# svohr/mixemt

Measured on AMD Instinct MI355X. Metric: read x hap cells/sec through the EM iteration (EM iters/sec reported beside it as em_iters_per_s), 1000000 reads x 5408 haps in total, whole job, higher is better.
Workload: dtype f64

## Files before the change

mixemt_amd/_lib.py:

```python

import ctypes
import os

_PKG = os.path.dirname(os.path.abspath(__file__))
LIB_PATH = os.environ.get("MXM_LIB") or os.path.join(_PKG, "lib", "libmixemt_hip.so")

c_i32, c_i64, c_f64 = ctypes.c_int32, ctypes.c_int64, ctypes.c_double
c_ptr, c_size = ctypes.c_void_p, ctypes.c_size_t


class EmState(ctypes.Structure):
    _fields_ = [("done", c_i32), ("iters", c_i32), ("l1", c_f64), ("ticket", ctypes.c_uint32), ("error", ctypes.c_uint32)]


class Coded(ctypes.Structure):
    _fields_ = [("rec", c_ptr), ("rec_off", c_ptr), ("ndist", c_ptr), ("R", c_i64),
                ("P_rest", c_ptr), ("ldp_rest", c_i64), ("w_rest", c_ptr), ("R_rest", c_i64),
                ("wide_rows", c_ptr), ("n_wide", c_i64),
                ("qrec", c_ptr), ("qoff", c_ptr), ("nquad", c_ptr), ("quad_rows", c_ptr), ("n_quad_rows", c_i64),
                ("byte_rows", c_ptr), ("n_byte_rows", c_i64)]


class SampleTile(ctypes.Structure):
    _fields_ = [("sample", c_i32), ("count", c_i32), ("first", c_i64)]
# ... 140 lines not shown
    "mxm_gather_columns": (ctypes.c_int, [c_ptr, c_i64, c_i64, c_i32, c_ptr, c_i32, c_ptr, c_i64, c_ptr]),
    "mxm_fold_logaddexp": (ctypes.c_int, [c_ptr, c_i64, ctypes.POINTER(c_ptr), ctypes.POINTER(c_i64), c_i32,
                                          c_i64, c_i32, c_f64, c_ptr]),
}

FINISH_SIGNATURES = {
    "mxm_samples_finish_workspace_bytes": (c_size, [c_i64, c_i32, c_i32]),
    "mxm_votes_samples": (ctypes.c_int, [ctypes.POINTER(Coded), c_ptr, c_i32, c_i32, c_ptr, c_ptr, c_ptr, c_ptr, c_ptr, c_ptr,
                                         c_ptr, c_ptr, c_ptr, c_ptr, c_ptr, c_size, c_ptr]),
    "mxm_gather_columns_samples": (ctypes.c_int, [ctypes.POINTER(Coded), c_ptr, c_i32, c_i32, c_ptr, c_ptr, c_i32, c_ptr,
                                                  c_ptr, c_size, c_ptr]),
    "mxm_em_loop_samples_narrow": (ctypes.c_int, [ctypes.POINTER(Coded), c_ptr, c_i32, c_i32, c_ptr, c_i32, c_ptr, c_ptr,
                                                  c_ptr, c_ptr, c_ptr, c_ptr, c_f64, c_i32, c_i32, c_ptr, c_ptr, c_size,
                                                  c_ptr, ctypes.POINTER(EmState)]),
    "mxm_assign_reads_samples": (ctypes.c_int, [ctypes.POINTER(Coded), c_ptr, c_i32, c_i32, c_ptr, c_i32, c_ptr, c_ptr,
                                                c_ptr, c_ptr, c_ptr, c_ptr, c_f64, c_ptr, c_ptr, c_ptr, c_size, c_ptr]),
}

VARCHECK_SIGNATURES = {
    "mxm_check_variants_samples": (ctypes.c_int, [c_ptr, c_i32, c_i64, c_ptr, c_ptr, c_i32, c_ptr, c_ptr, c_i32, c_i64, c_ptr,
                                                  c_ptr, c_i32, c_f64, c_f64, c_f64, c_i32, c_i32, c_ptr, c_ptr, c_ptr, c_ptr]),
}

ABI_VERSION = 603

PROGRESS_FN = ctypes.CFUNCTYPE(None, ctypes.POINTER(EmState), c_i32, c_ptr)

_lib = None


class MixemtHipError(RuntimeError):
    pass


def load():
    global _lib
    if _lib is not None:
        return _lib
    if not os.path.exists(LIB_PATH):
        raise MixemtHipError(
            "libmixemt_hip.so is not built (%s); run `python -m mixemt_amd.build` -- "
            "there is no CPU fallback for the EM hot path" % LIB_PATH)
    from . import _dev
    lib = ctypes.CDLL(LIB_PATH)
    try:
        lib.mxm_version.restype = ctypes.c_int
        lib.mxm_version.argtypes = []
        have = lib.mxm_version()
    except AttributeError:
        have = None
    if have != ABI_VERSION:
        raise MixemtHipError("%s reports ABI version %s, this binding was written for %d: rebuild with "
                             "`python -m mixemt_amd.build --force`" % (LIB_PATH, have, ABI_VERSION))
    for name, (restype, argtypes) in (list(SIGNATURES.items()) + list(FINISH_SIGNATURES.items())
                                      + list(VARCHECK_SIGNATURES.items())):
        try:
            fn = getattr(lib, name)
        except AttributeError:
            raise MixemtHipError("%s has ABI version %d but lacks %s: rebuild with "
                                 "`python -m mixemt_amd.build --force`" % (LIB_PATH, have, name))
        fn.restype = restype
        fn.argtypes = argtypes
    _lib = lib
    try:
        if _dev.torch is not None and _dev.torch.cuda.is_available():
            lib.mxm_preload()
    except Exception:
        pass
    return lib


def check(rc, what):
    if rc != 0:
        msg = load().mxm_last_error().decode("utf-8", "replace")
        raise ValueError("%s failed (%d): %s" % (what, rc, msg))
```

mixemt_amd/build.py:

```python

import hashlib
import os
import shutil
import subprocess
import sys

_PKG = os.path.dirname(os.path.abspath(__file__))
_ROOT = os.path.dirname(_PKG)
SRC = os.path.join(_PKG, "csrc", "mixemt_hip.hip")
HDRS = [os.path.join(_ROOT, "include", name) for name in ("mixemt_hip.h", "mixemt_hip_tuning.h", "mixemt_hip_samples_finish.h",
                                                           "mixemt_hip_var_check.h")]
LIB_DIR = os.path.join(_PKG, "lib")
LIB = os.path.join(LIB_DIR, "libmixemt_hip.so")
ARCH = "gfx950"


def _hipcc():
    for cand in (os.environ.get("HIPCC"), shutil.which("hipcc"), "/opt/rocm/bin/hipcc"):
        if cand and os.path.exists(cand):
            return cand
    raise RuntimeError("hipcc not found (set HIPCC or add /opt/rocm/bin to PATH)")


def _sources():
    csrc = os.path.dirname(SRC)
    return sorted(os.path.join(csrc, f) for f in os.listdir(csrc) if f.endswith((".hip", ".hpp"))) + HDRS


def _digest(flags):
    h = hashlib.sha256()
    for path in _sources():
        with open(path, "rb") as fin:
            h.update(fin.read())
    h.update(" ".join(flags).encode())
# ... 44 lines not shown
```

mixemt_amd/csrc/build_lut_kernels.hpp:

```cpp
#ifndef MIXEMT_BUILD_LUT_KERNELS_HPP
#define MIXEMT_BUILD_LUT_KERNELS_HPP

#define LUT_THREADS 256
#define LUT_CAP 128
#define LUT_NOMATCH (15u << 3)
#ifndef LUT_CPL
#define LUT_CPL 4
#endif
#ifndef LUT_UNROLL
#define LUT_UNROLL 8
#endif
#ifndef LUT_PIPE
#define LUT_PIPE 0
#endif

template <int NT, int CPL>
__global__ __launch_bounds__(LUT_THREADS) void build_lut_kernel(
    const uint8_t *__restrict__ E, int64_t lde, int64_t e_bytes, const double *__restrict__ lhit,
    const double *__restrict__ lmiss, const uint8_t *__restrict__ obsmap, const int64_t *__restrict__ row_ptr,
    const uint16_t *__restrict__ site, const uint8_t *__restrict__ obs, const int64_t *__restrict__ order,
    int64_t R, int H, double *__restrict__ M, int64_t ldm, int vec_ok, int compact) {
    static_assert(CPL == 4 || CPL == 8, "one 4- or 8-byte table load per lane, site and tile");
    constexpr int EW = CPL / 4;
    __shared__ double s_lut[2][LUT_CAP][16];
    __shared__ uint2 s_rec[2][LUT_CAP];
    const int t = threadIdx.x;
    const auto e_rsrc = __builtin_amdgcn_make_buffer_rsrc(const_cast<uint8_t *>(E), 0, (int)e_bytes, 0x00020000);

    auto stage = [&](int buf, int slot, int64_t at) {
        const uint32_t s0 = site[at];
        const uint32_t oc = obsmap[obs[at]];
        const double hv = lhit[s0], mv = lmiss[s0];
        s_rec[buf][slot] = make_uint2((uint32_t)(s0 * (uint32_t)lde), oc * 0x01010101u);
        d2 *dst = reinterpret_cast<d2 *>(&s_lut[buf][slot][0]);
        dst[0] = d2{hv, mv};
#pragma unroll
        for (int q = 1; q < 8; ++q) dst[q] = d2{mv, mv};
    };

    int cur = 0;
    bool have = false;
    for (int64_t i = blockIdx.x; i < R; i += gridDim.x, cur ^= 1) {
        const int64_t r = order != nullptr ? order[i] : i;
        const int64_t beg = row_ptr[r], end = row_ptr[r + 1];
// ... 117 lines not shown
```

mixemt_amd/csrc/coded_kernels.hpp:

```cpp
#ifndef MIXEMT_CODED_KERNELS_HPP
#define MIXEMT_CODED_KERNELS_HPP

#define ENC_THREADS 256
#define ENC_SLOTS 1024
#define ENC_MAX_CODES 256
#define ENC_MAX_WIDE 1024
#define ENC_WIDE_SLOTS 4096
#define ENC_EMPTY 0xFFFFFFFFFFFFFFFFull

__host__ __device__ __forceinline__ int rec_code_bytes(int nd, int ldc) { return nd > ENC_MAX_CODES ? 2 * ldc : ldc; }
__device__ __forceinline__ int rec_code_at(const uint8_t *codes, int h, bool wide) {
    return wide ? (int)reinterpret_cast<const uint16_t *>(codes)[h] : (int)codes[h];
}

template <int NCH, bool WIDE>
__device__ __forceinline__ void encode_one_row(int64_t r, const double *__restrict__ M, int64_t ldm, int H, int ldc,
                                               uint8_t *__restrict__ rec, int64_t rec_cap, int64_t *__restrict__ rec_off,
                                               int32_t *__restrict__ ndist, double *__restrict__ rowmax,
                                               unsigned long long *__restrict__ stats) {
    constexpr int NW = ENC_THREADS / 64;
    constexpr int SLOTS = WIDE ? ENC_WIDE_SLOTS : ENC_SLOTS;
    constexpr int MAXC = WIDE ? ENC_MAX_WIDE : ENC_MAX_CODES;
    constexpr int SPT = SLOTS / ENC_THREADS;
    __shared__ unsigned long long s_key[SLOTS];
    __shared__ unsigned short s_code[SLOTS];
    __shared__ double s_red[NW];
    __shared__ int s_wcnt[NW];
    __shared__ int s_flag, s_n;
    __shared__ long long s_off;
    const int t = threadIdx.x, lane = t & 63, wv = t >> 6;
    typedef unsigned int u4 __attribute__((ext_vector_type(4)));
    typedef unsigned int u2 __attribute__((ext_vector_type(2)));

    const auto rsrc = __builtin_amdgcn_make_buffer_rsrc(const_cast<double *>(M + r * ldm), 0, H * 8, 0x00020000);
    double x[NCH][4];
#pragma unroll
    for (int k = 0; k < NCH; ++k) {
        const int off = (t + k * ENC_THREADS) * 32;
        const d2 a = __builtin_bit_cast(d2, (u4)__builtin_amdgcn_raw_buffer_load_b128(rsrc, off, 0, 2));
// ... 122 lines not shown
        }
#pragma unroll
        for (int k = 0; k < NCH; ++k) {
            const int c0 = 4 * (t + k * ENC_THREADS);
            if (c0 < ldc) {
                unsigned int cd[4];
#pragma unroll
                for (int e = 0; e < 4; ++e) cd[e] = (c0 + e < H) ? (unsigned int)s_code[slot[k][e]] : 0u;
                if constexpr (WIDE) {
                    u2 word;
                    word.x = cd[0] | (cd[1] << 16);
                    word.y = cd[2] | (cd[3] << 16);
                    reinterpret_cast<u2 *>(rec + off)[t + k * ENC_THREADS] = word;
                } else {
                    reinterpret_cast<unsigned int *>(rec + off)[t + k * ENC_THREADS] =
                        cd[0] | (cd[1] << 8) | (cd[2] << 16) | (cd[3] << 24);
                }
            }
        }
    }
    if (t == 0) {
        if constexpr (WIDE) {
            if (off >= 0) {
                ndist[r] = D;
                rec_off[r] = off;
                atomicAdd(&stats[1], ~0ull);
            }
        } else {
            rowmax[r] = shift;
            ndist[r] = (off >= 0) ? D : 0;
            rec_off[r] = (off >= 0) ? off : 0;
            if (off < 0) atomicAdd(&stats[1], 1ull);
        }
    }
    __syncthreads();
}

template <int NCH>
__global__ __launch_bounds__(ENC_THREADS) void encode_rows_kernel(
    const double *__restrict__ M, int64_t ldm, int64_t R, int H, int ldc, uint8_t *__restrict__ rec, int64_t rec_cap,
    int64_t *__restrict__ rec_off, int32_t *__restrict__ ndist, double *__restrict__ rowmax,
    unsigned long long *__restrict__ stats) {
    for (int64_t r = blockIdx.x; r < R; r += gridDim.x)
        encode_one_row<NCH, false>(r, M, ldm, H, ldc, rec, rec_cap, rec_off, ndist, rowmax, stats);
}

template <int NCH>
__global__ __launch_bounds__(ENC_THREADS) void encode_wide_rows_kernel(
    const double *__restrict__ M, int64_t ldm, int64_t R, int H, int ldc, uint8_t *__restrict__ rec, int64_t rec_cap,
    int64_t *__restrict__ rec_off, int32_t *__restrict__ ndist, double *__restrict__ rowmax,
    unsigned long long *__restrict__ stats) {
    constexpr int CH = 32;
    __shared__ int s_list[CH];
    __shared__ int s_nlist;
    const int t = threadIdx.x;
    const int64_t nchunk = (R + CH - 1) / CH;
    for (int64_t c = blockIdx.x; c < nchunk; c += gridDim.x) {
        if (t == 0) s_nlist = 0;
        __syncthreads();
        const int64_t r = c * CH + t;
        if (t < CH && r < R && ndist[r] == 0) s_list[atomicAdd(&s_nlist, 1)] = t;
        __syncthreads();
        const int n = s_nlist;
        for (int i = 0; i < n; ++i)
            encode_one_row<NCH, true>(c * CH + s_list[i], M, ldm, H, ldc, rec, rec_cap, rec_off, ndist, rowmax, stats);
        __syncthreads();
    }
}

template <int THREADS, int NCH, int NBUF, bool NT, bool RESIDENT, bool WIDE_PREFETCH, bool CHECK = false>
__device__ __forceinline__ void coded_row_pass(const uint8_t *__restrict__ rec, const int64_t *__restrict__ rec_off,
                                               const int32_t *__restrict__ ndist, int ldc, const double *__restrict__ w,
                                               const int64_t *__restrict__ wide_rows, int64_t n_wide, int64_t R,
                                               const double (&p)[NCH][4], double (&acc)[NCH][4], bool &meta_ready,
                                               int *chk_result = nullptr, const int64_t *__restrict__ row_list = nullptr,
                                               int64_t n_list = 0, const int32_t *__restrict__ nquad = nullptr, int vbid = -1,
                                               int vgrid = 0) {
    static_assert(NBUF >= 3, "codes NBUF - 1 rows ahead, tables NBUF - 2");
    constexpr int NW = THREADS / 64;
    constexpr int AUX = NT ? 2 : 0;
    __shared__ double s_tbl[NBUF][ENC_MAX_CODES];
    __shared__ __attribute__((aligned(16))) double red[NBUF][NW];
    const int t = threadIdx.x, lane = t & 63, wv = t >> 6;
    const int nword = ldc >> 2;
    const int64_t bid = vbid >= 0 ? (int64_t)vbid : (int64_t)blockIdx.x, grid = vbid >= 0 ? (int64_t)vgrid : (int64_t)gridDim.x;
    const row_deal deal(row_list != nullptr ? n_list : R, bid, grid);
    const int voff = t * 4;
    int last_w = t + (NCH - 1) * THREADS;
// ... 474 lines not shown
```

mixemt_amd/csrc/mixemt_hip.hip:

```cpp
#include <hip/hip_runtime.h>
#include <stdint.h>
#include <stdio.h>
#include <stdlib.h>
#include <string.h>
#include <math.h>
#include <algorithm>
#include <atomic>
#include <mutex>
#include <type_traits>
#include <utility>
#include <vector>

#include "mixemt_hip.h"
#include "mixemt_hip_tuning.h"

#include "common.hpp"
#include "aln_encode.hpp"
#include "bam_reader.hpp"
#include "coded_kernels.hpp"
#include "quad_kernels.hpp"
#include "quad_batched_kernels.hpp"
#include "build_kernels.hpp"
#include "build_lut_kernels.hpp"
#include "build_sparse_kernels.hpp"
#include "em_kernels.hpp"
#include "estep_kernels.hpp"
#include "aux_kernels.hpp"
#include "records_kernels.hpp"
#include "fused_kernels.hpp"
#include "fused_cols_kernels.hpp"
#include "fused_coded_kernels.hpp"
#include "fused_narrow_kernels.hpp"
#include "samples_kernels.hpp"
#include "samples_finish_kernels.hpp"
#include "exchange.hpp"
#include "aln_walk.hpp"
#include "observe_kernels.hpp"
// ... 141 lines not shown
}

extern "C" int mxm_build_em_matrix(const uint8_t *E, int64_t lde, const double *lhit,
                                   const double *lmiss, const int64_t *row_ptr, const uint16_t *site,
                                   const uint8_t *obs, int64_t R, int32_t H, int32_t S, double *M,
                                   int64_t ldm, void *stream) {
    if (R < 0 || H <= 0 || S <= 0) return fail(-1, "mxm_build_em_matrix: bad shape R=%lld H=%d", (long long)R, H);
    if (lde < (((int64_t)H + 7) & ~(int64_t)7) || (lde & 7) != 0 || (reinterpret_cast<uintptr_t>(E) & 7) != 0)
        return fail(-1, "mxm_build_em_matrix: E must be 8-byte aligned with lde a multiple of 8 and >= H rounded up to 8 (lde=%lld)", (long long)lde);
    if (ldm < H) return fail(-1, "mxm_build_em_matrix: ldm < H");
    if (S > 65536) return fail(-1, "mxm_build_em_matrix: more than 65536 variant sites");
    if (R == 0) return 0;
    const int grid = clamp_grid(R, num_cu() * 8);
    const int vec_ok = ((ldm & 1) == 0) && ((reinterpret_cast<uintptr_t>(M) & 15) == 0);
    hipLaunchKernelGGL(build_em_matrix_kernel, dim3(grid), dim3(BUILD_THREADS), 0, (hipStream_t)stream, E,
                       lde, lhit, lmiss, row_ptr, site, obs, R, (int)H, M, ldm, vec_ok);
    HIP_TRY(hipGetLastError());
    return 0;
}

static int build_lut_impl(const char *who, const uint8_t *Ecode, int64_t lde, const double *lhit,
                          const double *lmiss, const uint8_t *obsmap, const int64_t *row_ptr, const uint16_t *site,
                          const uint8_t *obs, const int64_t *order, int64_t R, int32_t H, int32_t S, double *M, int64_t ldm,
                          int compact, hipStream_t s) {
    if (H > 8192) return fail(-1, "%s: more than 8192 haplogroups (H=%d)%s", who, H, compact ? "" : ": use mxm_build_em_matrix");
    if (lde < (((int64_t)H + 7) & ~(int64_t)7) || (lde & 7) != 0 || (reinterpret_cast<uintptr_t>(Ecode) & 7) != 0)
        return fail(-1, "%s: Ecode must be 8-byte aligned with lde a multiple of 8 and >= H rounded up to 8 (lde=%lld)", who, (long long)lde);
    if (ldm < H) return fail(-1, "%s: ldm < H", who);
    if (S > 65536 || (int64_t)S * lde >= ((int64_t)1 << 31))
        return fail(-1, "%s: table of %d x %lld bytes exceeds one buffer descriptor", who, S, (long long)lde);
    if (R == 0) return 0;
    const int grid = clamp_grid(R, num_cu() * 8);
    const int nt = (H + LUT_THREADS * LUT_CPL - 1) / (LUT_THREADS * LUT_CPL);
    const int vec_ok = ((ldm & 1) == 0) && ((reinterpret_cast<uintptr_t>(M) & 15) == 0);
    const bool ok = dispatch_width<8>(nt, [&](auto n) {
        constexpr int NT = decltype(n)::value;
        hipLaunchKernelGGL((build_lut_kernel<NT, LUT_CPL>), dim3(grid), dim3(LUT_THREADS), 0, s, Ecode, lde, (int64_t)S * lde, lhit,
                           lmiss, obsmap, row_ptr, site, obs, order, R, (int)H, M, ldm, vec_ok, compact);
    });
    if (!ok) return fail(-1, "%s: H=%d outside the kernel's range", who, H);
    HIP_TRY(hipGetLastError());
    return 0;
}

extern "C" int mxm_build_em_matrix_lut(const uint8_t *Ecode, int64_t lde, const double *lhit, const double *lmiss,
                                       const uint8_t *obsmap, const int64_t *row_ptr, const uint16_t *site,
                                       const uint8_t *obs, const int64_t *order, int64_t R, int32_t H, int32_t S,
                                       double *M, int64_t ldm, void *stream) {
    if (R < 0 || H <= 0 || S <= 0) return fail(-1, "mxm_build_em_matrix_lut: bad shape R=%lld H=%d", (long long)R, H);
    return build_lut_impl("mxm_build_em_matrix_lut", Ecode, lde, lhit, lmiss, obsmap, row_ptr, site, obs,
                          order, R, H, S, M, ldm, 0, (hipStream_t)stream);
}

extern "C" int mxm_build_em_matrix_lut_rows(const uint8_t *Ecode, int64_t lde, const double *lhit, const double *lmiss,
                                            const uint8_t *obsmap, const int64_t *row_ptr, const uint16_t *site,
                                            const uint8_t *obs, const int64_t *rows, int64_t n_rows, int32_t H, int32_t S,
                                            double *M_out, int64_t ldm, void *stream) {
    if (n_rows < 0 || H <= 0 || S <= 0 || rows == nullptr) return fail(-1, "mxm_build_em_matrix_lut_rows: bad arguments");
    return build_lut_impl("mxm_build_em_matrix_lut_rows", Ecode, lde, lhit, lmiss, obsmap, row_ptr, site, obs, rows, n_rows, H, S,
                          M_out, ldm, 1, (hipStream_t)stream);
}
// ... 115 lines not shown

extern "C" int mxm_build_em_records(const uint8_t *maj, const double *lhit, const double *lmiss,
                                    const int32_t *mk_ptr, const uint16_t *mk_hap, const uint8_t *mk_base,
                                    const int64_t *row_ptr, const uint16_t *site, const uint8_t *obs,
                                    const int64_t *order, int64_t R, int32_t H, int32_t S, double *M, int64_t ldm,
                                    uint8_t *rec, size_t rec_bytes, int64_t *rec_off, int32_t *ndist, double *rowmax,
                                    int64_t *stats, int64_t *fallback, int64_t *n_fallback, void *stream) {
    MXM_ENTER();
    if (!mxm_linear_supported(H))
        return fail(-1, "mxm_build_em_records: records need H in [65, 8192] (H=%d)", H);
    if (rec == nullptr || (reinterpret_cast<uintptr_t>(rec) & 15) || rec_bytes < (size_t)coded_ld(H) + 16 * ENC_MAX_CODES ||
        rec_off == nullptr || ndist == nullptr || rowmax == nullptr || stats == nullptr)
        return fail(-1, "mxm_build_em_records: record buffer (16-byte aligned, >= one record) and output arrays required");
    spb_records out;
    out.rec = rec;
    out.rec_cap = (long long)rec_bytes;
    out.rec_off = rec_off;
    out.ndist = ndist;
    out.rowmax = rowmax;
    out.stats = reinterpret_cast<unsigned long long *>(stats);
    out.ldc = coded_ld(H);
    return build_sparse_impl("mxm_build_em_records", maj, lhit, lmiss, mk_ptr, mk_hap, mk_base, row_ptr, site, obs, order,
                             R, H, S, M, ldm, &out, fallback, n_fallback, (hipStream_t)stream);
}

template <typename ST>
static int linearize_wide(const double *M, int64_t ldm, int64_t R, int H, ST *P, int64_t ldp, double *rowmax,
                          hipStream_t s) {
    const int nch = (H / 2 + 255) / 256;
    int cap = num_cu() * 2 < MXM_MAX_WG ? num_cu() * 2 : MXM_MAX_WG;
    const int nwg = clamp_grid((R + 1) / 2, cap);
    const bool ok = dispatch_width<16>(nch, [&](auto n) {
        hipLaunchKernelGGL((linearize_wide_kernel<decltype(n)::value, ST>), dim3(nwg), dim3(256), 0, s, M, ldm, R, H, P, ldp, rowmax);
    });
    return ok ? 0 : 1;
}

static inline bool wide_rows_ok(const void *M, int64_t ldm, int H) {
    return ((H & 1) == 0) && ((ldm & 1) == 0) && ((reinterpret_cast<uintptr_t>(M) & 15) == 0) && H >= 64 && H <= 8192;
}

extern "C" int mxm_linearize(const double *M, int64_t ldm, int64_t R, int32_t H, double *P, int64_t ldp,
                             double *rowmax, void *stream) {
    if (R < 0 || H <= 0) return fail(-1, "mxm_linearize: bad shape");
    if (ldm < H || ldp < H || (ldp & 1)) return fail(-1, "mxm_linearize: ldp must be even and >= H (ldp=%lld)", (long long)ldp);
    if (R == 0) return 0;
// ... 2168 lines not shown
```

mixemt_amd/preprocess.py:

```python

import collections
import math
import os
import sys
import time

import numpy

from . import _lib
from . import phylotree
from ._dev import as_device, current_stream, device_empty, require_gpu, to_host, torch

MUT_WT = 0.01
MUT_MAX = 0.5


class _LazyLut(object):

    def __init__(self, expected, n_haps, code_of, obsmap):
        self._expected, self._n_haps, self.code_of = expected, n_haps, code_of
        self._items = {"obsmap": obsmap}

    def __getitem__(self, key):
        if key == "ecode" and "ecode" not in self._items:
# ... 252 lines not shown
    return torch.argsort(keys, stable=True)


def build_em_matrix_device(tables, row_ptr, site, obs, out=None, kernel="auto", sort_rows="auto"):
    lib = _lib.load()
    dev = require_gpu()
    if kernel == "auto":
        kernel = "bytes" if tables.lut() is None else "sparse"
    if kernel not in ("sparse", "lut", "bytes"):
        raise ValueError("kernel must be 'auto', 'sparse', 'lut' or 'bytes'")
    if kernel == "sparse":
        if tables.lut() is None or tables.n_haps > 8192:
            raise ValueError("tables do not qualify for the marker kernel (its leftover rows need the lookup-table kernel)")
        enc = tables.sparse_device()
        row_ptr_d = as_device(row_ptr, torch.int64, dev)
        site_d = as_device(site, torch.uint16, dev)
        obs_d = as_device(obs, torch.uint8, dev)
        n_rows = row_ptr_d.numel() - 1
        n_haps = tables.n_haps
        if out is None:
            out = device_empty((n_rows, n_haps), torch.float64, dev, "the EM input matrix")
        if n_rows == 0:
            return out
        fallback = torch.empty(n_rows, dtype=torch.int64, device=dev)
        n_fallback = torch.zeros(1, dtype=torch.int64, device=dev)
        _lib.check(lib.mxm_build_em_matrix_sparse(
            enc["maj"].data_ptr(), enc["lhit"].data_ptr(), enc["lmiss"].data_ptr(), enc["mk_ptr"].data_ptr(),
            enc["mk_hap"].data_ptr(), enc["mk_base"].data_ptr(), row_ptr_d.data_ptr(), site_d.data_ptr(),
            obs_d.data_ptr(), 0, n_rows, n_haps, len(tables.sites), out.data_ptr(), out.stride(0),
            fallback.data_ptr(), n_fallback.data_ptr(), current_stream()), "mxm_build_em_matrix_sparse")
        left = int(n_fallback.item())
        build_em_matrix_device.last_fallback = left
        if left:
            lut = tables.lut_device()
            rows = fallback[:left].sort().values
            _lib.check(lib.mxm_build_em_matrix_lut(
                lut["ecode"].data_ptr(), lut["ecode"].stride(0), lut["lhit"].data_ptr(), lut["lmiss"].data_ptr(),
                lut["obsmap"].data_ptr(), row_ptr_d.data_ptr(), site_d.data_ptr(), obs_d.data_ptr(),
                rows.data_ptr(), left, n_haps, len(tables.sites), out.data_ptr(), out.stride(0),
                current_stream()), "mxm_build_em_matrix_lut")
        return out
    if kernel == "lut":
        enc = tables.lut_device()
        if enc is None:
            raise ValueError("tables do not qualify for the lookup-table kernel")
        row_ptr_d = as_device(row_ptr, torch.int64, dev)
        site_d = as_device(site, torch.uint16, dev)
        obs_d = as_device(obs, torch.uint8, dev)
        n_rows = row_ptr_d.numel() - 1
        n_haps = tables.n_haps
        if out is None:
            out = device_empty((n_rows, n_haps), torch.float64, dev, "the EM input matrix")
        if n_rows == 0:
            return out
        order = None
        if sort_rows is True or (sort_rows == "auto" and n_rows >= SORT_ROWS_FROM):
            order = row_order_by_position(row_ptr_d, site_d)
        _lib.check(lib.mxm_build_em_matrix_lut(
            enc["ecode"].data_ptr(), enc["ecode"].stride(0), enc["lhit"].data_ptr(), enc["lmiss"].data_ptr(),
            enc["obsmap"].data_ptr(), row_ptr_d.data_ptr(), site_d.data_ptr(), obs_d.data_ptr(),
            0 if order is None else order.data_ptr(), n_rows, n_haps, len(tables.sites),
            out.data_ptr(), out.stride(0), current_stream()), "mxm_build_em_matrix_lut")
        return out
# ... 157 lines not shown
        raise ValueError("records need tables that qualify for the lookup-table kernel and H in [65, 8192]")
    enc = tables.sparse_device()
    lut = tables.lut_device()
    row_ptr_d = as_device(row_ptr, torch.int64, dev)
    site_d = as_device(site, torch.uint16, dev)
    obs_d = as_device(obs, torch.uint8, dev)
    n_rows, n_haps, n_sites = row_ptr_d.numel() - 1, tables.n_haps, len(tables.sites)
    if n_rows <= 0:
        raise ValueError("no rows")
    ldc = (n_haps + 7) // 8 * 8
    worst = lib.mxm_record_bytes(n_rows, n_haps)
    one = 2 * ldc + 16 * 1024
    if rec is not None and (rec.dtype != torch.uint8 or not rec.is_cuda or rec.numel() < one or rec.data_ptr() % 16):
        rec = None
    if rec is not None:
        cap = rec.numel()
    elif cap is None:
        cap = record_buffer_bytes(n_rows, n_haps, mean_sites=site_d.numel() / float(n_rows))
    cap = max(int(cap), one)
    mat = device_empty((n_rows, n_haps), torch.float64, dev, "the EM input matrix") if dense else None
    rec_off = torch.empty(n_rows, dtype=torch.int64, device=dev)
    ndist = torch.empty(n_rows, dtype=torch.int32, device=dev)
    rowmax = torch.empty(n_rows, dtype=torch.float64, device=dev)
    counters = torch.zeros(5, dtype=torch.int64, device=dev)
    stats, n_fallback, sub_stats = counters[0:2], counters[2:3], counters[3:5]
    fallback = torch.empty(n_rows, dtype=torch.int64, device=dev)
    stream = current_stream()
    timing = {} if os.environ.get("MXM_PIPELINE_TIMING") else None
    build_em_records_device.last_timing = timing

    def lap(name, t0):
        if timing is not None:
            torch.cuda.synchronize()
            timing[name] = round(timing.get(name, 0.0) + (time.perf_counter() - t0) * 1e3, 2)
        return time.perf_counter()

    def lut_rows(rows_d, count, out):
        _lib.check(lib.mxm_build_em_matrix_lut_rows(
            lut["ecode"].data_ptr(), lut["ecode"].stride(0), lut["lhit"].data_ptr(), lut["lmiss"].data_ptr(),
            lut["obsmap"].data_ptr(), row_ptr_d.data_ptr(), site_d.data_ptr(), obs_d.data_ptr(), rows_d.data_ptr(), count,
            n_haps, n_sites, out.data_ptr(), out.stride(0), stream), "mxm_build_em_matrix_lut_rows")

    for attempt in (0, 1):
        t_lap = lap("uploads", time.perf_counter()) if attempt == 0 and timing is not None else time.perf_counter()
        if rec is None:
            rec = device_empty((cap,), torch.uint8, dev, "the coded matrix")
        _lib.check(lib.mxm_build_em_records(
            enc["maj"].data_ptr(), enc["lhit"].data_ptr(), enc["lmiss"].data_ptr(), enc["mk_ptr"].data_ptr(),
            enc["mk_hap"].data_ptr(), enc["mk_base"].data_ptr(), row_ptr_d.data_ptr(), site_d.data_ptr(), obs_d.data_ptr(),
            0, n_rows, n_haps, n_sites, mat.data_ptr() if dense else 0, mat.stride(0) if dense else 0,
            rec.data_ptr(), cap, rec_off.data_ptr(), ndist.data_ptr(), rowmax.data_ptr(), stats.data_ptr(),
            fallback.data_ptr(), n_fallback.data_ptr(), stream), "mxm_build_em_records")
        used, n_rest, left = (int(v) for v in counters[:3].cpu())
        t_lap = lap("marker kernel", t_lap)
        need = used
        m_rest = None
        rest_rows = fallback[:0]
        if used <= cap:
            if dense:
                if left:
                    rows = fallback[:left].sort().values
                    _lib.check(lib.mxm_build_em_matrix_lut(
                        lut["ecode"].data_ptr(), lut["ecode"].stride(0), lut["lhit"].data_ptr(), lut["lmiss"].data_ptr(),
                        lut["obsmap"].data_ptr(), row_ptr_d.data_ptr(), site_d.data_ptr(), obs_d.data_ptr(), rows.data_ptr(), left,
                        n_haps, n_sites, mat.data_ptr(), mat.stride(0), stream), "mxm_build_em_matrix_lut")
                rest_rows = torch.nonzero(ndist == 0).flatten()
                assert rest_rows.numel() == n_rest
            else:
                assert left == n_rest
                if n_rest:
                    rest_host = numpy.sort(fallback[:left].cpu().numpy())
                    rest_rows = torch.from_numpy(rest_host).to(dev)
                    t_lap = lap("list sort", t_lap)
            if n_rest:
                slab = min(n_rest, REST_SLAB_ROWS if REST_SLAB_ROWS else max(1024, REST_SLAB_BYTES // (8 * n_haps)))
                m_slab = None if dense else torch.empty((slab, n_haps), dtype=torch.float64, device=dev)
                sub_off = torch.empty(slab, dtype=torch.int64, device=dev)
                sub_nd = torch.empty(slab, dtype=torch.int32, device=dev)
                sub_rm = torch.empty(slab, dtype=torch.float64, device=dev)
                kept_rows, kept_dense, kept_host = [], [], []
                for lo in range(0, n_rest, slab):
                    rows_s = rest_rows[lo:lo + slab]
                    n_s = int(rows_s.numel())
                    if dense:
                        m_s = mat.index_select(0, rows_s)
                    else:
                        m_s = m_slab[:n_s]
                        lut_rows(rows_s, n_s, m_s)
                        t_lap = lap("slab build", t_lap)
                    base = (need + 15) // 16 * 16
                    room = cap - base >= one
                    if room:
                        _lib.check(lib.mxm_encode_rows(m_s.data_ptr(), m_s.stride(0), n_s, n_haps, rec.data_ptr() + base,
                                                       cap - base, sub_off.data_ptr(), sub_nd.data_ptr(), sub_rm.data_ptr(),
                                                       sub_stats.data_ptr(), stream), "mxm_encode_rows")
                        sub_used, sub_left = (int(v) for v in sub_stats.cpu())
                        t_lap = lap("slab encode", t_lap)
                    else:
                        sub_used, sub_left = n_s * one, 0
                    if room and base + sub_used <= cap:
                        _lib.check(lib.mxm_scatter_records(rows_s.data_ptr(), n_s, sub_off.data_ptr(), sub_nd.data_ptr(),
                                                           sub_rm.data_ptr(), base, rec_off.data_ptr(), ndist.data_ptr(),
                                                           rowmax.data_ptr(), stream), "mxm_scatter_records")
                        if sub_left:
                            if dense:
                                got = sub_nd[:n_s] > 0
                                kept_rows.append(rows_s[~got])
                                kept_dense.append(m_s[~got].clone())
                            else:
                                kept_host.append(rest_host[lo:lo + n_s][sub_nd[:n_s].cpu().numpy() == 0])
                        t_lap = lap("slab scatter / keep", t_lap)
                    need = base + sub_used
                if need <= cap:
                    used = need
                    if dense:
                        rest_rows = torch.cat(kept_rows) if kept_rows else rest_rows[:0]
                        m_rest = torch.cat(kept_dense) if kept_dense else None
                    elif kept_host:
                        kept = numpy.concatenate(kept_host)
                        rest_rows = torch.from_numpy(kept).to(dev)
                        m_rest = torch.empty((len(kept), n_haps), dtype=torch.float64, device=dev)
                        lut_rows(rest_rows, len(kept), m_rest)
                        t_lap = lap("kept rows", t_lap)
                    else:
                        rest_rows = rest_rows[:0]
                    n_rest = int(rest_rows.numel())
        if need <= cap:
            break
        if attempt == 1:
            raise ValueError("build_em_records_device: record buffer of %d bytes overflowed twice (%d needed)" % (cap, need))
        rec = None
        cap = min(worst, need + (n_rest + 1) * one)
    build_em_matrix_device.last_fallback = left
    cm = CodedMatrix(n_rows, n_haps, rec, rec_off, ndist, rowmax, used,
                     rest_rows, m_rest if m_rest is not None else torch.empty((0, n_haps), dtype=torch.float64, device=dev))
    cm.capacity = cap
    return (cm, mat) if dense else cm


def build_em_records_many(tables, samples_csr, cap=None):
    if not samples_csr:
        raise ValueError("no samples")
    ptrs, sites, obss, row0, nnz = [], [], [], [0], 0
    for row_ptr, site, obs in samples_csr:
        rp = numpy.asarray(row_ptr.cpu() if isinstance(row_ptr, torch.Tensor) else row_ptr, dtype=numpy.int64)
        if rp.ndim != 1 or rp.size < 2 or rp[0] != 0:
            raise ValueError("every sample needs at least one row (row_ptr[0] = 0)")
        ptrs.append(rp[(1 if ptrs else 0):] + nnz)
        nnz += int(rp[-1])
# ... 150 lines not shown
```

Baseline: 882.0 billion.

## Fuse leftover-row LUT build and encoding into device-side record build pass

Adds fused C entry points that run the sparse marker build, then the LUT build and encoding of the fallback rows, all on device. The kernels read the fallback count from device memory, so the host no longer has to sync, sort the row list and loop over slabs with several readbacks. Leftover rows are encoded through a listed-row kernel that writes straight into the global record arrays, which removes the separate scatter step. The cost is more complex kernels with device-side bounds. Slab processing now follows fallback-list order instead of sorted row order, which may hurt memory locality.

Result: no change. 878.5 billion, median of 2 (-0.4%).

```diff
diff --git a/include/mixemt_hip_build.h b/include/mixemt_hip_build.h
--- /dev/null
+++ b/include/mixemt_hip_build.h
@@ -0,0 +1,37 @@
+#ifndef MIXEMT_HIP_BUILD_H
+#define MIXEMT_HIP_BUILD_H
+
+#include <stddef.h>
+#include <stdint.h>
+
+#ifdef __cplusplus
+extern "C" {
+#endif
+
+int mxm_build_em_matrix_sparse_lut(const uint8_t *maj, const double *lhit, const double *lmiss,
+                                   const int32_t *mk_ptr, const uint16_t *mk_hap, const uint8_t *mk_base,
+                                   const uint8_t *Ecode, int64_t lde, const uint8_t *obsmap,
+                                   const int64_t *row_ptr, const uint16_t *site, const uint8_t *obs,
+                                   const int64_t *order, int64_t R, int32_t H, int32_t S,
+                                   double *M, int64_t ldm, int64_t *fallback, int64_t *n_fallback, void *stream);
+
+int mxm_finish_em_records(const uint8_t *Ecode, int64_t lde, const double *lhit, const double *lmiss,
+                          const uint8_t *obsmap, const int64_t *row_ptr, const uint16_t *site, const uint8_t *obs,
+                          int32_t H, int32_t S, double *M, int64_t ldm, double *slab, int64_t ld_slab, int64_t slab_rows,
+                          int64_t first, uint8_t *rec, size_t rec_bytes, int64_t *rec_off, int32_t *ndist, double *rowmax,
+                          int64_t *stats, const int64_t *fallback, const int64_t *n_fallback, void *stream);
+
+int mxm_build_em_records_all(const uint8_t *maj, const double *lhit, const double *lmiss,
+                             const int32_t *mk_ptr, const uint16_t *mk_hap, const uint8_t *mk_base,
+                             const uint8_t *Ecode, int64_t lde, const uint8_t *obsmap,
+                             const int64_t *row_ptr, const uint16_t *site, const uint8_t *obs,
+                             const int64_t *order, int64_t R, int32_t H, int32_t S, double *M, int64_t ldm,
+                             double *slab, int64_t ld_slab, int64_t slab_rows,
+                             uint8_t *rec, size_t rec_bytes, int64_t *rec_off, int32_t *ndist, double *rowmax,
+                             int64_t *stats, int64_t *fallback, int64_t *n_fallback, void *stream);
+
+#ifdef __cplusplus
+}
+#endif
+
+#endif
diff --git a/mixemt_amd/_lib.py b/mixemt_amd/_lib.py
--- a/mixemt_amd/_lib.py
+++ b/mixemt_amd/_lib.py
@@ -186,6 +186,17 @@
                                                   c_ptr, c_i32, c_f64, c_f64, c_f64, c_i32, c_i32, c_ptr, c_ptr, c_ptr, c_ptr]),
 }
 
+BUILD_SIGNATURES = {
+    "mxm_build_em_matrix_sparse_lut": (ctypes.c_int, [c_ptr, c_ptr, c_ptr, c_ptr, c_ptr, c_ptr, c_ptr, c_i64, c_ptr, c_ptr, c_ptr,
+                                                      c_ptr, c_ptr, c_i64, c_i32, c_i32, c_ptr, c_i64, c_ptr, c_ptr, c_ptr]),
+    "mxm_finish_em_records": (ctypes.c_int, [c_ptr, c_i64, c_ptr, c_ptr, c_ptr, c_ptr, c_ptr, c_ptr, c_i32, c_i32, c_ptr, c_i64,
+                                             c_ptr, c_i64, c_i64, c_i64, c_ptr, c_size, c_ptr, c_ptr, c_ptr, c_ptr, c_ptr, c_ptr,
+                                             c_ptr]),
+    "mxm_build_em_records_all": (ctypes.c_int, [c_ptr, c_ptr, c_ptr, c_ptr, c_ptr, c_ptr, c_ptr, c_i64, c_ptr, c_ptr, c_ptr, c_ptr,
+                                                c_ptr, c_i64, c_i32, c_i32, c_ptr, c_i64, c_ptr, c_i64, c_i64, c_ptr, c_size,
+                                                c_ptr, c_ptr, c_ptr, c_ptr, c_ptr, c_ptr, c_ptr]),
+}
+
 ABI_VERSION = 603
 
 PROGRESS_FN = ctypes.CFUNCTYPE(None, ctypes.POINTER(EmState), c_i32, c_ptr)
@@ -217,7 +228,7 @@
         raise MixemtHipError("%s reports ABI version %s, this binding was written for %d: rebuild with "
                              "`python -m mixemt_amd.build --force`" % (LIB_PATH, have, ABI_VERSION))
     for name, (restype, argtypes) in (list(SIGNATURES.items()) + list(FINISH_SIGNATURES.items())
-                                      + list(VARCHECK_SIGNATURES.items())):
+                                      + list(VARCHECK_SIGNATURES.items()) + list(BUILD_SIGNATURES.items())):
         try:
             fn = getattr(lib, name)
         except AttributeError:
diff --git a/mixemt_amd/build.py b/mixemt_amd/build.py
--- a/mixemt_amd/build.py
+++ b/mixemt_amd/build.py
@@ -9,7 +9,7 @@
 _ROOT = os.path.dirname(_PKG)
 SRC = os.path.join(_PKG, "csrc", "mixemt_hip.hip")
 HDRS = [os.path.join(_ROOT, "include", name) for name in ("mixemt_hip.h", "mixemt_hip_tuning.h", "mixemt_hip_samples_finish.h",
-                                                           "mixemt_hip_var_check.h")]
+                                                           "mixemt_hip_var_check.h", "mixemt_hip_build.h")]
 LIB_DIR = os.path.join(_PKG, "lib")
 LIB = os.path.join(LIB_DIR, "libmixemt_hip.so")
 ARCH = "gfx950"
diff --git a/mixemt_amd/csrc/build_lut_kernels.hpp b/mixemt_amd/csrc/build_lut_kernels.hpp
--- a/mixemt_amd/csrc/build_lut_kernels.hpp
+++ b/mixemt_amd/csrc/build_lut_kernels.hpp
@@ -19,7 +19,13 @@
     const uint8_t *__restrict__ E, int64_t lde, int64_t e_bytes, const double *__restrict__ lhit,
     const double *__restrict__ lmiss, const uint8_t *__restrict__ obsmap, const int64_t *__restrict__ row_ptr,
     const uint16_t *__restrict__ site, const uint8_t *__restrict__ obs, const int64_t *__restrict__ order,
-    int64_t R, int H, double *__restrict__ M, int64_t ldm, int vec_ok, int compact) {
+    int64_t R, int H, double *__restrict__ M, int64_t ldm, int vec_ok, int compact,
+    const unsigned long long *__restrict__ n_dev, int64_t first) {
+    if (n_dev != nullptr) {
+        const int64_t left = (int64_t)*n_dev - first;
+        R = left < 0 ? 0 : (left < R ? left : R);
+        order += first;
+    }
     static_assert(CPL == 4 || CPL == 8, "one 4- or 8-byte table load per lane, site and tile");
     constexpr int EW = CPL / 4;
     __shared__ double s_lut[2][LUT_CAP][16];
diff --git a/mixemt_amd/csrc/coded_kernels.hpp b/mixemt_amd/csrc/coded_kernels.hpp
--- a/mixemt_amd/csrc/coded_kernels.hpp
+++ b/mixemt_amd/csrc/coded_kernels.hpp
@@ -13,8 +13,8 @@
     return wide ? (int)reinterpret_cast<const uint16_t *>(codes)[h] : (int)codes[h];
 }
 
-template <int NCH, bool WIDE>
-__device__ __forceinline__ void encode_one_row(int64_t r, const double *__restrict__ M, int64_t ldm, int H, int ldc,
+template <int NCH, bool WIDE, bool LISTED = false>
+__device__ __forceinline__ void encode_one_row(int64_t r, int64_t r_out, const double *__restrict__ M, int64_t ldm, int H, int ldc,
                                                uint8_t *__restrict__ rec, int64_t rec_cap, int64_t *__restrict__ rec_off,
                                                int32_t *__restrict__ ndist, double *__restrict__ rowmax,
                                                unsigned long long *__restrict__ stats) {
@@ -183,15 +183,21 @@
     if (t == 0) {
         if constexpr (WIDE) {
             if (off >= 0) {
-                ndist[r] = D;
-                rec_off[r] = off;
+                ndist[r_out] = D;
+                rec_off[r_out] = off;
                 atomicAdd(&stats[1], ~0ull);
+            } else if constexpr (LISTED) {
+                rowmax[r_out] = 0.0;
             }
         } else {
-            rowmax[r] = shift;
-            ndist[r] = (off >= 0) ? D : 0;
-            rec_off[r] = (off >= 0) ? off : 0;
-            if (off < 0) atomicAdd(&stats[1], 1ull);
+            rowmax[r_out] = shift;
+            ndist[r_out] = (off >= 0) ? D : 0;
+            rec_off[r_out] = (off >= 0) ? off : 0;
+            if constexpr (LISTED) {
+                if (off >= 0) atomicAdd(&stats[1], ~0ull);
+            } else {
+                if (off < 0) atomicAdd(&stats[1], 1ull);
+            }
         }
     }
     __syncthreads();
@@ -203,7 +209,7 @@
     int64_t *__restrict__ rec_off, int32_t *__restrict__ ndist, double *__restrict__ rowmax,
     unsigned long long *__restrict__ stats) {
     for (int64_t r = blockIdx.x; r < R; r += gridDim.x)
-        encode_one_row<NCH, false>(r, M, ldm, H, ldc, rec, rec_cap, rec_off, ndist, rowmax, stats);
+        encode_one_row<NCH, false>(r, r, M, ldm, H, ldc, rec, rec_cap, rec_off, ndist, rowmax, stats);
 }
 
 template <int NCH>
@@ -224,7 +230,50 @@
         __syncthreads();
         const int n = s_nlist;
         for (int i = 0; i < n; ++i)
-            encode_one_row<NCH, true>(c * CH + s_list[i], M, ldm, H, ldc, rec, rec_cap, rec_off, ndist, rowmax, stats);
+            encode_one_row<NCH, true>(c * CH + s_list[i], c * CH + s_list[i], M, ldm, H, ldc, rec, rec_cap, rec_off, ndist, rowmax, stats);
+        __syncthreads();
+    }
+}
+
+template <int NCH>
+__global__ __launch_bounds__(ENC_THREADS) void encode_listed_rows_kernel(
+    const double *__restrict__ M, int64_t ldm, int compact, const int64_t *__restrict__ rows,
+    const unsigned long long *__restrict__ n_dev, int64_t first, int64_t cap_rows, int H, int ldc, uint8_t *__restrict__ rec,
+    int64_t rec_cap, int64_t *__restrict__ rec_off, int32_t *__restrict__ ndist, double *__restrict__ rowmax,
+    unsigned long long *__restrict__ stats) {
+    const int64_t left = (int64_t)*n_dev - first;
+    const int64_t n = left < 0 ? 0 : (left < cap_rows ? left : cap_rows);
+    for (int64_t i = blockIdx.x; i < n; i += gridDim.x) {
+        const int64_t r = rows[first + i];
+        encode_one_row<NCH, false, true>(compact ? i : r, r, M, ldm, H, ldc, rec, rec_cap, rec_off, ndist, rowmax, stats);
+    }
+}
+
+template <int NCH>
+__global__ __launch_bounds__(ENC_THREADS) void encode_wide_listed_rows_kernel(
+    const double *__restrict__ M, int64_t ldm, int compact, const int64_t *__restrict__ rows,
+    const unsigned long long *__restrict__ n_dev, int64_t first, int64_t cap_rows, int H, int ldc, uint8_t *__restrict__ rec,
+    int64_t rec_cap, int64_t *__restrict__ rec_off, int32_t *__restrict__ ndist, double *__restrict__ rowmax,
+    unsigned long long *__restrict__ stats) {
+    constexpr int CH = 32;
+    __shared__ int s_list[CH];
+    __shared__ int s_nlist;
+    const int t = threadIdx.x;
+    const int64_t left = (int64_t)*n_dev - first;
+    const int64_t n = left < 0 ? 0 : (left < cap_rows ? left : cap_rows);
+    const int64_t nchunk = (n + CH - 1) / CH;
+    for (int64_t c = blockIdx.x; c < nchunk; c += gridDim.x) {
+        if (t == 0) s_nlist = 0;
+        __syncthreads();
+        const int64_t i = c * CH + t;
+        if (t < CH && i < n && ndist[rows[first + i]] == 0) s_list[atomicAdd(&s_nlist, 1)] = t;
+        __syncthreads();
+        const int m = s_nlist;
+        for (int e = 0; e < m; ++e) {
+            const int64_t at = c * CH + s_list[e];
+            const int64_t r = rows[first + at];
+            encode_one_row<NCH, true, true>(compact ? at : r, r, M, ldm, H, ldc, rec, rec_cap, rec_off, ndist, rowmax, stats);
+        }
         __syncthreads();
     }
 }
diff --git a/mixemt_amd/csrc/mixemt_hip.hip b/mixemt_amd/csrc/mixemt_hip.hip
--- a/mixemt_amd/csrc/mixemt_hip.hip
+++ b/mixemt_amd/csrc/mixemt_hip.hip
@@ -13,6 +13,7 @@
 
 #include "mixemt_hip.h"
 #include "mixemt_hip_tuning.h"
+#include "mixemt_hip_build.h"
 
 #include "common.hpp"
 #include "aln_encode.hpp"
@@ -200,21 +201,22 @@
 static int build_lut_impl(const char *who, const uint8_t *Ecode, int64_t lde, const double *lhit,
                           const double *lmiss, const uint8_t *obsmap, const int64_t *row_ptr, const uint16_t *site,
                           const uint8_t *obs, const int64_t *order, int64_t R, int32_t H, int32_t S, double *M, int64_t ldm,
-                          int compact, hipStream_t s) {
+                          int compact, hipStream_t s, const int64_t *n_dev = nullptr, int64_t first = 0, bool check_only = false) {
     if (H > 8192) return fail(-1, "%s: more than 8192 haplogroups (H=%d)%s", who, H, compact ? "" : ": use mxm_build_em_matrix");
     if (lde < (((int64_t)H + 7) & ~(int64_t)7) || (lde & 7) != 0 || (reinterpret_cast<uintptr_t>(Ecode) & 7) != 0)
         return fail(-1, "%s: Ecode must be 8-byte aligned with lde a multiple of 8 and >= H rounded up to 8 (lde=%lld)", who, (long long)lde);
     if (ldm < H) return fail(-1, "%s: ldm < H", who);
     if (S > 65536 || (int64_t)S * lde >= ((int64_t)1 << 31))
         return fail(-1, "%s: table of %d x %lld bytes exceeds one buffer descriptor", who, S, (long long)lde);
-    if (R == 0) return 0;
+    if (R == 0 || check_only) return 0;
     const int grid = clamp_grid(R, num_cu() * 8);
     const int nt = (H + LUT_THREADS * LUT_CPL - 1) / (LUT_THREADS * LUT_CPL);
     const int vec_ok = ((ldm & 1) == 0) && ((reinterpret_cast<uintptr_t>(M) & 15) == 0);
     const bool ok = dispatch_width<8>(nt, [&](auto n) {
         constexpr int NT = decltype(n)::value;
         hipLaunchKernelGGL((build_lut_kernel<NT, LUT_CPL>), dim3(grid), dim3(LUT_THREADS), 0, s, Ecode, lde, (int64_t)S * lde, lhit,
-                           lmiss, obsmap, row_ptr, site, obs, order, R, (int)H, M, ldm, vec_ok, compact);
+                           lmiss, obsmap, row_ptr, site, obs, order, R, (int)H, M, ldm, vec_ok, compact,
+                           reinterpret_cast<const unsigned long long *>(n_dev), first);
     });
     if (!ok) return fail(-1, "%s: H=%d outside the kernel's range", who, H);
     HIP_TRY(hipGetLastError());
@@ -376,6 +378,118 @@
     out.ldc = coded_ld(H);
     return build_sparse_impl("mxm_build_em_records", maj, lhit, lmiss, mk_ptr, mk_hap, mk_base, row_ptr, site, obs, order,
                              R, H, S, M, ldm, &out, fallback, n_fallback, (hipStream_t)stream);
+}
+
+extern "C" int mxm_build_em_matrix_sparse_lut(const uint8_t *maj, const double *lhit, const double *lmiss,
+                                              const int32_t *mk_ptr, const uint16_t *mk_hap, const uint8_t *mk_base,
+                                              const uint8_t *Ecode, int64_t lde, const uint8_t *obsmap,
+                                              const int64_t *row_ptr, const uint16_t *site, const uint8_t *obs,
+                                              const int64_t *order, int64_t R, int32_t H, int32_t S, double *M, int64_t ldm,
+                                              int64_t *fallback, int64_t *n_fallback, void *stream) {
+    MXM_ENTER();
+    const char *who = "mxm_build_em_matrix_sparse_lut";
+    if (M == nullptr) return fail(-1, "%s: M required", who);
+    if (R < 0 || H <= 0 || S <= 0) return fail(-1, "%s: bad shape R=%lld H=%d", who, (long long)R, H);
+    if (Ecode == nullptr || obsmap == nullptr) return fail(-1, "%s: the lookup tables of the leftover rows are required", who);
+    int rc = build_lut_impl(who, Ecode, lde, lhit, lmiss, obsmap, row_ptr, site, obs, fallback, R, H, S, M, ldm, 0,
+                            (hipStream_t)stream, n_fallback, 0, true);
+    if (rc != 0) return rc;
+    rc = build_sparse_impl(who, maj, lhit, lmiss, mk_ptr, mk_hap, mk_base, row_ptr, site, obs, order, R, H, S, M, ldm, nullptr,
+                           fallback, n_fallback, (hipStream_t)stream);
+    if (rc != 0) return rc;
+    return build_lut_impl(who, Ecode, lde, lhit, lmiss, obsmap, row_ptr, site, obs, fallback, R, H, S, M, ldm, 0,
+                          (hipStream_t)stream, n_fallback, 0);
+}
+
+static int finish_records_impl(const char *who, const uint8_t *Ecode, int64_t lde, const double *lhit, const double *lmiss,
+                               const uint8_t *obsmap, const int64_t *row_ptr, const uint16_t *site, const uint8_t *obs,
+                               int32_t H, int32_t S, double *M, int64_t ldm, double *slab, int64_t ld_slab, int64_t slab_rows,
+                               int64_t first, const spb_records &out, const int64_t *fallback, const int64_t *n_fallback,
+                               hipStream_t s, bool check_only) {
+    if (Ecode == nullptr || obsmap == nullptr || fallback == nullptr || n_fallback == nullptr)
+        return fail(-1, "%s: the lookup tables and the list of leftover rows are required", who);
+    if (slab_rows < 0 || first < 0) return fail(-1, "%s: bad slab_rows=%lld first=%lld", who, (long long)slab_rows, (long long)first);
+    if (M == nullptr && slab_rows > 0 && (slab == nullptr || ld_slab < H || (reinterpret_cast<uintptr_t>(slab) & 7) != 0))
+        return fail(-1, "%s: without a dense matrix the leftover rows need a slab (8-byte aligned, ld_slab >= H)", who);
+    const int compact = M == nullptr ? 1 : 0;
+    double *dense = compact ? slab : M;
+    const int64_t ldd = compact ? ld_slab : ldm;
+    int rc = build_lut_impl(who, Ecode, lde, lhit, lmiss, obsmap, row_ptr, site, obs, fallback, slab_rows, H, S, dense, ldd, compact,
+                            s, n_fallback, first, check_only);
+    if (rc != 0 || check_only || slab_rows == 0) return rc;
+    const int ldc = coded_ld(H);
+    const int nch = (ldc / 4 + ENC_THREADS - 1) / ENC_THREADS;
+    const int grid = clamp_grid(slab_rows, num_cu() * 4);
+    const int grid_w = clamp_grid((slab_rows + 31) / 32, num_cu() * 3);
+    const unsigned long long *n_dev = reinterpret_cast<const unsigned long long *>(n_fallback);
+    const bool ok = dispatch_width<8>(nch, [&](auto n) {
+        constexpr int NCH = decltype(n)::value;
+        hipLaunchKernelGGL((encode_listed_rows_kernel<NCH>), dim3(grid), dim3(ENC_THREADS), 0, s, dense, ldd, compact, fallback, n_dev,
+                           first, slab_rows, (int)H, ldc, out.rec, (int64_t)out.rec_cap, out.rec_off, out.ndist, out.rowmax, out.stats);
+        hipLaunchKernelGGL((encode_wide_listed_rows_kernel<NCH>), dim3(grid_w), dim3(ENC_THREADS), 0, s, dense, ldd, compact, fallback,
+                           n_dev, first, slab_rows, (int)H, ldc, out.rec, (int64_t)out.rec_cap, out.rec_off, out.ndist, out.rowmax,
+                           out.stats);
+    });
+    if (!ok) return fail(-1, "%s: H=%d outside the encoder's range", who, H);
+    HIP_TRY(hipGetLastError());
+    return 0;
+}
+
+static int records_out(const char *who, int32_t H, uint8_t *rec, size_t rec_bytes, int64_t *rec_off, int32_t *ndist, double *rowmax,
+                       int64_t *stats, spb_records *out) {
+    if (!mxm_linear_supported(H)) return fail(-1, "%s: records need H in [65, 8192] (H=%d)", who, H);
+    if (rec == nullptr || (reinterpret_cast<uintptr_t>(rec) & 15) || rec_bytes < (size_t)coded_ld(H) + 16 * ENC_MAX_CODES ||
+        rec_off == nullptr || ndist == nullptr || rowmax == nullptr || stats == nullptr)
+        return fail(-1, "%s: record buffer (16-byte aligned, >= one record) and output arrays required", who);
+    out->rec = rec;
+    out->rec_cap = (long long)rec_bytes;
+    out->rec_off = rec_off;
+    out->ndist = ndist;
+    out->rowmax = rowmax;
+    out->stats = reinterpret_cast<unsigned long long *>(stats);
+    out->ldc = coded_ld(H);
+    return 0;
+}
+
+extern "C" int mxm_finish_em_records(const uint8_t *Ecode, int64_t lde, const double *lhit, const double *lmiss,
+                                     const uint8_t *obsmap, const int64_t *row_ptr, const uint16_t *site, const uint8_t *obs,
+                                     int32_t H, int32_t S, double *M, int64_t ldm, double *slab, int64_t ld_slab,
+                                     int64_t slab_rows, int64_t first, uint8_t *rec, size_t rec_bytes, int64_t *rec_off,
+                                     int32_t *ndist, double *rowmax, int64_t *stats, const int64_t *fallback,
+                                     const int64_t *n_fallback, void *stream) {
+    MXM_ENTER();
+    const char *who = "mxm_finish_em_records";
+    if (H <= 0 || S <= 0) return fail(-1, "%s: bad shape H=%d S=%d", who, H, S);
+    spb_records out;
+    const int rc = records_out(who, H, rec, rec_bytes, rec_off, ndist, rowmax, stats, &out);
+    if (rc != 0) return rc;
+    return finish_records_impl(who, Ecode, lde, lhit, lmiss, obsmap, row_ptr, site, obs, H, S, M, ldm, slab, ld_slab, slab_rows, first,
+                               out, fallback, n_fallback, (hipStream_t)stream, false);
+}
+
+extern "C" int mxm_build_em_records_all(const uint8_t *maj, const double *lhit, const double *lmiss,
+                                        const int32_t *mk_ptr, const uint16_t *mk_hap, const uint8_t *mk_base,
+                                        const uint8_t *Ecode, int64_t lde, const uint8_t *obsmap,
+                                        const int64_t *row_ptr, const uint16_t *site, const uint8_t *obs,
+                                        const int64_t *order, int64_t R, int32_t H, int32_t S, double *M, int64_t ldm,
+                                        double *slab, int64_t ld_slab, int64_t slab_rows,
+                                        uint8_t *rec, size_t rec_bytes, int64_t *rec_off, int32_t *ndist, double *rowmax,
+                                        int64_t *stats, int64_t *fallback, int64_t *n_fallback, void *stream) {
+    MXM_ENTER();
+    const char *who = "mxm_build_em_records_all";
+    if (R < 0 || H <= 0 || S <= 0) return fail(-1, "%s: bad shape R=%lld H=%d", who, (long long)R, H);
+    spb_records out;
+    int rc = records_out(who, H, rec, rec_bytes, rec_off, ndist, rowmax, stats, &out);
+    if (rc != 0) return rc;
+    if (M != nullptr && ldm < H) return fail(-1, "%s: ldm < H", who);
+    rc = finish_records_impl(who, Ecode, lde, lhit, lmiss, obsmap, row_ptr, site, obs, H, S, M, ldm, slab, ld_slab, slab_rows, 0, out,
+                             fallback, n_fallback, (hipStream_t)stream, true);
+    if (rc != 0) return rc;
+    rc = build_sparse_impl(who, maj, lhit, lmiss, mk_ptr, mk_hap, mk_base, row_ptr, site, obs, order, R, H, S, M, ldm, &out, fallback,
+                           n_fallback, (hipStream_t)stream);
+    if (rc != 0 || R == 0) return rc;
+    return finish_records_impl(who, Ecode, lde, lhit, lmiss, obsmap, row_ptr, site, obs, H, S, M, ldm, slab, ld_slab, slab_rows, 0, out,
+                               fallback, n_fallback, (hipStream_t)stream, false);
 }
 
 template <typename ST>
diff --git a/mixemt_amd/preprocess.py b/mixemt_amd/preprocess.py
--- a/mixemt_amd/preprocess.py
+++ b/mixemt_amd/preprocess.py
@@ -298,23 +298,16 @@
             out = device_empty((n_rows, n_haps), torch.float64, dev, "the EM input matrix")
         if n_rows == 0:
             return out
+        lut = tables.lut_device()
         fallback = torch.empty(n_rows, dtype=torch.int64, device=dev)
-        n_fallback = torch.zeros(1, dtype=torch.int64, device=dev)
-        _lib.check(lib.mxm_build_em_matrix_sparse(
+        n_fallback = torch.empty(1, dtype=torch.int64, device=dev)
+        _lib.check(lib.mxm_build_em_matrix_sparse_lut(
             enc["maj"].data_ptr(), enc["lhit"].data_ptr(), enc["lmiss"].data_ptr(), enc["mk_ptr"].data_ptr(),
-            enc["mk_hap"].data_ptr(), enc["mk_base"].data_ptr(), row_ptr_d.data_ptr(), site_d.data_ptr(),
-            obs_d.data_ptr(), 0, n_rows, n_haps, len(tables.sites), out.data_ptr(), out.stride(0),
-            fallback.data_ptr(), n_fallback.data_ptr(), current_stream()), "mxm_build_em_matrix_sparse")
-        left = int(n_fallback.item())
-        build_em_matrix_device.last_fallback = left
-        if left:
-            lut = tables.lut_device()
-            rows = fallback[:left].sort().values
-            _lib.check(lib.mxm_build_em_matrix_lut(
-                lut["ecode"].data_ptr(), lut["ecode"].stride(0), lut["lhit"].data_ptr(), lut["lmiss"].data_ptr(),
-                lut["obsmap"].data_ptr(), row_ptr_d.data_ptr(), site_d.data_ptr(), obs_d.data_ptr(),
-                rows.data_ptr(), left, n_haps, len(tables.sites), out.data_ptr(), out.stride(0),
-                current_stream()), "mxm_build_em_matrix_lut")
+            enc["mk_hap"].data_ptr(), enc["mk_base"].data_ptr(), lut["ecode"].data_ptr(), lut["ecode"].stride(0),
+            lut["obsmap"].data_ptr(), row_ptr_d.data_ptr(), site_d.data_ptr(), obs_d.data_ptr(), 0, n_rows, n_haps,
+            len(tables.sites), out.data_ptr(), out.stride(0), fallback.data_ptr(), n_fallback.data_ptr(), current_stream()),
+            "mxm_build_em_matrix_sparse_lut")
+        build_em_matrix_device.last_fallback = int(n_fallback.item())
         return out
     if kernel == "lut":
         enc = tables.lut_device()
@@ -518,9 +511,12 @@
     rec_off = torch.empty(n_rows, dtype=torch.int64, device=dev)
     ndist = torch.empty(n_rows, dtype=torch.int32, device=dev)
     rowmax = torch.empty(n_rows, dtype=torch.float64, device=dev)
-    counters = torch.zeros(5, dtype=torch.int64, device=dev)
-    stats, n_fallback, sub_stats = counters[0:2], counters[2:3], counters[3:5]
+    counters = torch.zeros(3, dtype=torch.int64, device=dev)
+    stats, n_fallback = counters[0:2], counters[2:3]
     fallback = torch.empty(n_rows, dtype=torch.int64, device=dev)
+    slab_rows = min(n_rows, REST_SLAB_ROWS if REST_SLAB_ROWS else max(1024, REST_SLAB_BYTES // (8 * n_haps)))
+    m_slab = None if dense else torch.empty((slab_rows, n_haps), dtype=torch.float64, device=dev)
+    take = n_rows if dense else slab_rows
     stream = current_stream()
     timing = {} if os.environ.get("MXM_PIPELINE_TIMING") else None
     build_em_records_device.last_timing = timing
@@ -541,86 +537,39 @@
         t_lap = lap("uploads", time.perf_counter()) if attempt == 0 and timing is not None else time.perf_counter()
         if rec is None:
             rec = device_empty((cap,), torch.uint8, dev, "the coded matrix")
-        _lib.check(lib.mxm_build_em_records(
+        _lib.check(lib.mxm_build_em_records_all(
             enc["maj"].data_ptr(), enc["lhit"].data_ptr(), enc["lmiss"].data_ptr(), enc["mk_ptr"].data_ptr(),
-            enc["mk_hap"].data_ptr(), enc["mk_base"].data_ptr(), row_ptr_d.data_ptr(), site_d.data_ptr(), obs_d.data_ptr(),
+            enc["mk_hap"].data_ptr(), enc["mk_base"].data_ptr(), lut["ecode"].data_ptr(), lut["ecode"].stride(0),
+            lut["obsmap"].data_ptr(), row_ptr_d.data_ptr(), site_d.data_ptr(), obs_d.data_ptr(),
             0, n_rows, n_haps, n_sites, mat.data_ptr() if dense else 0, mat.stride(0) if dense else 0,
+            0 if dense else m_slab.data_ptr(), 0 if dense else m_slab.stride(0), take,
             rec.data_ptr(), cap, rec_off.data_ptr(), ndist.data_ptr(), rowmax.data_ptr(), stats.data_ptr(),
-            fallback.data_ptr(), n_fallback.data_ptr(), stream), "mxm_build_em_records")
-        used, n_rest, left = (int(v) for v in counters[:3].cpu())
-        t_lap = lap("marker kernel", t_lap)
+            fallback.data_ptr(), n_fallback.data_ptr(), stream), "mxm_build_em_records_all")
+        used, n_rest, left = (int(v) for v in counters.cpu())
+        t_lap = lap("build and leftover rows", t_lap)
+        if left > take:
+            for first in range(take, left, take):
+                _lib.check(lib.mxm_finish_em_records(
+                    lut["ecode"].data_ptr(), lut["ecode"].stride(0), lut["lhit"].data_ptr(), lut["lmiss"].data_ptr(),
+                    lut["obsmap"].data_ptr(), row_ptr_d.data_ptr(), site_d.data_ptr(), obs_d.data_ptr(), n_haps, n_sites,
+                    0, 0, m_slab.data_ptr(), m_slab.stride(0), take, first, rec.data_ptr(), cap, rec_off.data_ptr(),
+                    ndist.data_ptr(), rowmax.data_ptr(), stats.data_ptr(), fallback.data_ptr(), n_fallback.data_ptr(), stream),
+                    "mxm_finish_em_records")
+            used, n_rest = (int(v) for v in stats.cpu())
+            t_lap = lap("further slabs", t_lap)
         need = used
         m_rest = None
         rest_rows = fallback[:0]
-        if used <= cap:
+        if need <= cap and n_rest:
+            kept = numpy.flatnonzero(ndist.cpu().numpy() == 0)
+            assert len(kept) == n_rest, (len(kept), n_rest)
+            rest_rows = torch.from_numpy(kept).to(dev)
             if dense:
-                if left:
-                    rows = fallback[:left].sort().values
-                    _lib.check(lib.mxm_build_em_matrix_lut(
-                        lut["ecode"].data_ptr(), lut["ecode"].stride(0), lut["lhit"].data_ptr(), lut["lmiss"].data_ptr(),
-                        lut["obsmap"].data_ptr(), row_ptr_d.data_ptr(), site_d.data_ptr(), obs_d.data_ptr(), rows.data_ptr(), left,
-                        n_haps, n_sites, mat.data_ptr(), mat.stride(0), stream), "mxm_build_em_matrix_lut")
-                rest_rows = torch.nonzero(ndist == 0).flatten()
-                assert rest_rows.numel() == n_rest
+                m_rest = mat.index_select(0, rest_rows)
             else:
-                assert left == n_rest
-                if n_rest:
-                    rest_host = numpy.sort(fallback[:left].cpu().numpy())
-                    rest_rows = torch.from_numpy(rest_host).to(dev)
-                    t_lap = lap("list sort", t_lap)
-            if n_rest:
-                slab = min(n_rest, REST_SLAB_ROWS if REST_SLAB_ROWS else max(1024, REST_SLAB_BYTES // (8 * n_haps)))
-                m_slab = None if dense else torch.empty((slab, n_haps), dtype=torch.float64, device=dev)
-                sub_off = torch.empty(slab, dtype=torch.int64, device=dev)
-                sub_nd = torch.empty(slab, dtype=torch.int32, device=dev)
-                sub_rm = torch.empty(slab, dtype=torch.float64, device=dev)
-                kept_rows, kept_dense, kept_host = [], [], []
-                for lo in range(0, n_rest, slab):
-                    rows_s = rest_rows[lo:lo + slab]
-                    n_s = int(rows_s.numel())
-                    if dense:
-                        m_s = mat.index_select(0, rows_s)
-                    else:
-                        m_s = m_slab[:n_s]
-                        lut_rows(rows_s, n_s, m_s)
-                        t_lap = lap("slab build", t_lap)
-                    base = (need + 15) // 16 * 16
-                    room = cap - base >= one
-                    if room:
-                        _lib.check(lib.mxm_encode_rows(m_s.data_ptr(), m_s.stride(0), n_s, n_haps, rec.data_ptr() + base,
-                                                       cap - base, sub_off.data_ptr(), sub_nd.data_ptr(), sub_rm.data_ptr(),
-                                                       sub_stats.data_ptr(), stream), "mxm_encode_rows")
-                        sub_used, sub_left = (int(v) for v in sub_stats.cpu())
-                        t_lap = lap("slab encode", t_lap)
-                    else:
-                        sub_used, sub_left = n_s * one, 0
-                    if room and base + sub_used <= cap:
-                        _lib.check(lib.mxm_scatter_records(rows_s.data_ptr(), n_s, sub_off.data_ptr(), sub_nd.data_ptr(),
-                                                           sub_rm.data_ptr(), base, rec_off.data_ptr(), ndist.data_ptr(),
-                                                           rowmax.data_ptr(), stream), "mxm_scatter_records")
-                        if sub_left:
-                            if dense:
-                                got = sub_nd[:n_s] > 0
-                                kept_rows.append(rows_s[~got])
-                                kept_dense.append(m_s[~got].clone())
-                            else:
-                                kept_host.append(rest_host[lo:lo + n_s][sub_nd[:n_s].cpu().numpy() == 0])
-                        t_lap = lap("slab scatter / keep", t_lap)
-                    need = base + sub_used
-                if need <= cap:
-                    used = need
-                    if dense:
-                        rest_rows = torch.cat(kept_rows) if kept_rows else rest_rows[:0]
-                        m_rest = torch.cat(kept_dense) if kept_dense else None
-                    elif kept_host:
-                        kept = numpy.concatenate(kept_host)
-                        rest_rows = torch.from_numpy(kept).to(dev)
-                        m_rest = torch.empty((len(kept), n_haps), dtype=torch.float64, device=dev)
-                        lut_rows(rest_rows, len(kept), m_rest)
-                        t_lap = lap("kept rows", t_lap)
-                    else:
-                        rest_rows = rest_rows[:0]
-                    n_rest = int(rest_rows.numel())
+                m_rest = torch.empty((len(kept), n_haps), dtype=torch.float64, device=dev)
+                lut_rows(rest_rows, len(kept), m_rest)
+            t_lap = lap("kept rows", t_lap)
         if need <= cap:
             break
         if attempt == 1:
```
